# Keep-Passion/ImageStitch

Hardware: AMD Instinct MI355X
Metric: image-pairs/sec (2048x2048 grayscale, SURF+BF) (higher is better)
Workload: dtype f32

## Files before the change

### imagestitch_amd/csrc/api.hip

```cpp
#include "common.h"
#include "canvas_band.h"
#include "ingest_fill.h"
#include "jpeg_huff_core.h"
#include "phase_resolve_math.h"
#include <math.h>
#include <stdarg.h>
#include <stdio.h>
#include <string.h>
#include <algorithm>
#include <map>
#include <tuple>

int fuse_i64_device(vfsms_ctx *ctx, const long long *dA, const long long *dB, int r, int c, int ch, int dx, int dy,
                    uint8_t *d_out, int32_t *info, int method = 0, int levels = 4, int seam_blend = 0, int32_t *d_seam = nullptr);

static thread_local char g_err[512] = "";
void vfsms_set_error(const char *fmt, ...)
{
    va_list ap;
    va_start(ap, fmt);
    vsnprintf(g_err, sizeof(g_err), fmt, ap);
    va_end(ap);
}
extern "C" int vfsms_last_error(char *buf, int buflen)
// ... 747 lines not shown
    if (split > 0) surf_describe_layout(a, &W, cap0);
    if (split < n) surf_describe_layout(a, &W, cap1);
    return a.off;
}
static int surf_run_carve(vfsms_ctx *ctx, SurfRun *run, const SurfSrc *S, int n, const vfsms_surf_params *p, const SurfEnh &enh)
{
    ArenaWalk a = ctx_arena_walk(ctx);
    surf_run_layout(a, run, S, n, p, enh);
    TRY(ctx_arena_commit(ctx, a, "arena exhausted while carving a SURF run"));
    return ctx_copy_small(ctx, run->R.data(), sizeof(RoiDev) * n, run->dR);
}
static int surf_run_prepare(vfsms_ctx *ctx, SurfRun *run, const SurfEnh &enh)
{
    const int n = (int)run->R.size();
    if (enh.mode) {
        TRY(ctx_copy_small(ctx, run->E.data(), sizeof(EnhJob) * n, run->dE));
        TRY(launch_enhance(ctx, run->dE, run->E.data(), n, enh.mode, enh.clip_limit, enh.tile_grid));
    }
    HIP_TRY(hipMemsetAsync(run->cblock, 0, sizeof(int) * 16 * n, ctx->stream));
    return VFSMS_OK;
}
static int surf_run_launch(vfsms_ctx *ctx, const SurfRun &run, int first, int count, bool describe, const vfsms_surf_params *p)
{
    TRY(launch_surf_detect(ctx, run.dR + first, run.R.data() + first, count, p));
    if (describe) TRY(launch_surf_describe(ctx, run.dR + first, run.R.data() + first, count, p));
    return VFSMS_OK;
}
static int surf_run_readback(vfsms_ctx *ctx, SurfRun *run)
{
    run->counters.resize(16 * run->R.size());
    HIP_TRY(hipMemcpyAsync(run->counters.data(), run->cblock, sizeof(int) * run->counters.size(), hipMemcpyDeviceToHost, ctx->stream));
    return VFSMS_OK;
}
static int surf_run_check(const SurfRun &run, const char *who, const char *unit, int index0, int total)
{
    for (size_t i = 0; i < run.R.size(); i++)
        if (run.counters[16 * i + 2] || run.counters[16 * i] > run.R[i].cap) {
            vfsms_set_error("%s: %s %d of %d (%d x %d) exceeded %d keypoint candidates (raise with vfsms_ctx_set_keypoint_capacity)",
                            who, unit, index0 + (int)i, total, run.R[i].h, run.R[i].w, run.R[i].cap);
            return VFSMS_ERR_CAPACITY;
        }
    return VFSMS_OK;
}
static int surf_run_count(const SurfRun &run, int i) { return run.counters[16 * (size_t)i + 1]; }

static int surf_host(vfsms_ctx *ctx, const uint8_t *img, int h, int w, int stride, const vfsms_surf_params *params,
                     float *kps_xy, float *desc, vfsms_keypoint *kps_full, int cap, int *n_out, bool describe)
// ... 2152 lines not shown
```

### imagestitch_amd/csrc/common.h

```cpp
#pragma once
#include <hip/hip_runtime.h>
#include <stdint.h>
#include <condition_variable>
#include <list>
#include <mutex>
#include <string>
#include <unordered_map>
#include <vector>
#include "../../include/vfsms.h"
#include "arena_walk.h"
#include "device_buf.h"

#define VFSMS_MAX_LAYERS 32
#define VFSMS_MAX_WIN 768

#define VFSMS_MAX_OCTAVES 8
#ifdef __HIPCC__
__host__ __device__
#endif
constexpr int vfsms_haar_corner(int size, int k, int c)
{
    constexpr int src[10][4] = { {0, 2, 3, 7}, {3, 2, 6, 7}, {6, 2, 9, 7}, {2, 0, 7, 3}, {2, 3, 7, 6}, {2, 6, 7, 9},
                                 {1, 1, 4, 4}, {5, 1, 8, 4}, {1, 5, 4, 8}, {5, 5, 8, 8} };
    return (2 * size * src[k][c] + 9) / 18;
}
#ifdef __HIPCC__
__host__ __device__
#endif
constexpr int vfsms_haar_src(int k, int c)
{
    constexpr int src[10][4] = { {0, 2, 3, 7}, {3, 2, 6, 7}, {6, 2, 9, 7}, {2, 0, 7, 3}, {2, 3, 7, 6}, {2, 6, 7, 9},
                                 {1, 1, 4, 4}, {5, 1, 8, 4}, {1, 5, 4, 8}, {5, 5, 8, 8} };
    return src[k][c];
// ... 187 lines not shown
void *ctx_arena_alloc(vfsms_ctx *ctx, size_t bytes, size_t align = 256);
ArenaWalk ctx_arena_walk(vfsms_ctx *ctx);
int ctx_arena_commit(vfsms_ctx *ctx, const ArenaWalk &a, const char *what);
int ctx_prepare_surf(vfsms_ctx *ctx, const vfsms_surf_params *p);

struct ShapeRun { int first, count, h, w; };
template <typename Rec>
static std::vector<ShapeRun> shape_runs(const Rec *recs, int n)
{
    std::vector<ShapeRun> runs;
    for (int r = 0; r < n; r++) {
        if (!runs.empty() && runs.back().h == recs[r].h && runs.back().w == recs[r].w) runs.back().count++;
        else runs.push_back(ShapeRun{r, 1, recs[r].h, recs[r].w});
    }
    return runs;
}

void surf_roi_layout(ArenaWalk &a, RoiDev *r, const uint8_t *img, int stride, int h, int w, int cap, const vfsms_surf_params *p);
struct DescWork { int *tickets; DescPlan *plan; DescRec *rec_big, *rec_small; };
void surf_describe_layout(ArenaWalk &a, DescWork *d, size_t capsum);
int launch_integral(vfsms_ctx *ctx, const RoiDev *d_rois, int nrois, int maxh, int maxw);
size_t integral_carry_bytes(int h, int w);
int launch_surf_detect(vfsms_ctx *ctx, const RoiDev *d_rois, const RoiDev *h_rois, int nrois,
                       const vfsms_surf_params *p);
int launch_surf_describe(vfsms_ctx *ctx, const RoiDev *d_rois, const RoiDev *h_rois, int nrois,
                         const vfsms_surf_params *p);
void match_layout(ArenaWalk &a, MatchDev *m, int capq, int dim, int nsplit);
void match_filter_layout(ArenaWalk &a, MatchDev *m, int capq, int capt, int cns);
int launch_max_norm2_d64(vfsms_ctx *ctx, const float *a, int n, unsigned *d_out);
int launch_bf_l2_filtered(vfsms_ctx *ctx, const MatchDev *d_jobs, int njobs, int capq, int capt, int cns);
int launch_bf_l2(vfsms_ctx *ctx, const MatchDev *d_jobs, int njobs, int capq, int nsplit, int dim);
#define BFI_PAD_NORM 0x3fffffff
struct PackJob { const float *src; const int *n_ptr; int8_t *dst; int *nrm; };
int launch_pack_i8_d128(vfsms_ctx *ctx, const PackJob *d_jobs, int njobs, int max_rows);
int launch_bf_i8_d128(vfsms_ctx *ctx, const MatchDev *d_jobs, int njobs, int capq, int nsplit);
int launch_bf_hamming(vfsms_ctx *ctx, const MatchDev *d_jobs, int njobs, int capq, int nsplit, int max_dist);
enum MatchTailKind {
    TAIL_VOTE,
    TAIL_PAIRS,
    TAIL_KNN,
    TAIL_GIVEN_PAIRS
};
struct MatchTail {
    MatchTailKind kind;
    double ratio;
    int max_dist;
    int offset_evaluate;
// ... 196 lines not shown
```

### imagestitch_amd/csrc/surf_kernels.hip

```cpp
#include "common.h"
#include "detmath.h"
#include <math.h>
#include <float.h>
#include <string.h>
#include <stdlib.h>
#include <algorithm>
#include <vector>

#define GAS __attribute__((address_space(1)))
typedef GAS const uint8_t *g_cu8;
typedef GAS const int32_t *g_ci32;
typedef GAS float *g_f32;
typedef GAS const float *g_cf32;
typedef GAS int32_t *g_i32;
__device__ __forceinline__ int cv_round_f(float v) { return (int)rintf(v); }
__device__ __forceinline__ uint8_t round_u8_pos(float v) { return (uint8_t)__float_as_uint(v + 12582912.f); }
__device__ __forceinline__ int cv_round_d(double v) { return (int)rint(v); }
__device__ __forceinline__ int cv_floor_d(double v) { return (int)floor(v); }
__device__ __forceinline__ int cv_ceil_d(double v) { return (int)ceil(v); }

__device__ __forceinline__ int wave_incl_scan(int v)
{
    const int lane = threadIdx.x & 63;
#pragma unroll
    for (int d = 1; d < 64; d <<= 1) {
        int n = __shfl_up(v, d, 64);
        if (lane >= d) v += n;
    }
    return v;
}

#define INT_TH 16
typedef int int4u __attribute__((ext_vector_type(4), aligned(4)));
typedef uint32_t u32u __attribute__((aligned(1)));

__device__ __forceinline__ uint32_t load_px4(g_cu8 row, int x, int w)
{
    const int xa = min(x, w - 4);
    const uint32_t v = *(GAS const u32u *)(row + xa);
    return v >> (8 * (x - xa));
}

__global__ __launch_bounds__(256) void k_integral_bandsum(const RoiDev *rois)
{
    const RoiDev &R = rois[blockIdx.z];
    const int h = R.h, w = R.w, stride = R.stride, ipitch = R.ipitch;
    const int y0 = blockIdx.y * INT_TH;
    const int x = (blockIdx.x * 256 + threadIdx.x) * 4;
    if (y0 >= h || x >= w || w < 4) return;
    const int rows = min(INT_TH, h - y0);
    g_cu8 src = (g_cu8)R.img + (size_t)y0 * stride;
    g_i32 dst = (g_i32)R.icarry + (size_t)blockIdx.y * ipitch + x;
    uint32_t px[INT_TH];
#pragma unroll
    for (int r = 0; r < INT_TH; r++) px[r] = r < rows ? load_px4(src + (size_t)r * stride, x, w) : 0u;
    uint32_t even = 0, odd = 0;
#pragma unroll
    for (int r = 0; r < INT_TH; r++) { even += px[r] & 0x00ff00ffu; odd += (px[r] >> 8) & 0x00ff00ffu; }
    int4u o = {(int)(even & 0xffff), (int)(odd & 0xffff), (int)(even >> 16), (int)(odd >> 16)};
    *(GAS int4u *)dst = o;
}

__global__ __launch_bounds__(256) void k_integral_bandscan(const RoiDev *rois)
{
    const RoiDev &R = rois[blockIdx.y];
    const int ipitch = R.ipitch;
    const int x = blockIdx.x * 256 + threadIdx.x;
    if (x >= ipitch) return;
    const int nb = (R.h + INT_TH - 1) / INT_TH;
    g_i32 c = (g_i32)R.icarry + x;
    int run = 0;
    for (int b0 = 0; b0 < nb; b0 += 16) {
        int v[16];
#pragma unroll
        for (int k = 0; k < 16; k++) v[k] = b0 + k < nb ? c[(size_t)(b0 + k) * ipitch] : 0;
#pragma unroll
        for (int k = 0; k < 16; k++) { if (b0 + k < nb) c[(size_t)(b0 + k) * ipitch] = run; run += v[k]; }
    }
}

__global__ __launch_bounds__(256) void k_integral_final(const RoiDev *rois)
{
    const RoiDev &R = rois[blockIdx.y];
    const int h = R.h, w = R.w, stride = R.stride, ipitch = R.ipitch;
    g_cu8 img = (g_cu8)R.img;
    g_i32 S = (g_i32)R.sum;
    g_ci32 carry = (g_ci32)R.icarry + (size_t)blockIdx.x * ipitch;
    const int y0 = blockIdx.x * INT_TH;
    if (y0 >= h) return;
    const int rows = min(INT_TH, h - y0);
    const int sw = w + 1;
    if (w < 4) {
        if (blockIdx.x == 0 && threadIdx.x == 0) {
            for (int xx = 0; xx < sw; xx++) S[xx] = 0;
            for (int y = 0; y < h; y++) {
                int rs = 0;
                S[(size_t)(y + 1) * sw] = 0;
                for (int xx = 0; xx < w; xx++) { rs += img[(size_t)y * stride + xx]; S[(size_t)(y + 1) * sw + xx + 1] = S[(size_t)y * sw + xx + 1] + rs; }
            }
        }
        return;
    }
    if (blockIdx.x == 0)
        for (int xx = threadIdx.x; xx < sw; xx += 256) S[xx] = 0;
    if (threadIdx.x < rows) S[(size_t)(y0 + 1 + threadIdx.x) * sw] = 0;
    __shared__ int wsum[INT_TH][4];
    const int lane = threadIdx.x & 63, wid = threadIdx.x >> 6;
    g_cu8 src = img + (size_t)y0 * stride;
    int ccarry[INT_TH];
#pragma unroll
    for (int r = 0; r < INT_TH; r++) ccarry[r] = 0;
    for (int c0 = 0; c0 < w; c0 += 1024) {
        const int x = c0 + threadIdx.x * 4;
        const bool in = x < w;
        const int xl = in ? x : 0;
        uint32_t px[INT_TH];
#pragma unroll
        for (int r = 0; r < INT_TH; r++) {
            const uint32_t v = load_px4(src + (size_t)min(r, rows - 1) * stride, xl, w);
            px[r] = (in && r < rows) ? v : 0u;
        }
        int4u C = *(GAS const int4u *)(carry + xl);
        if (!in) { C.x = 0; C.y = 0; C.z = 0; C.w = 0; }
        int tot[INT_TH];
        int run = C.x + C.y + C.z + C.w;
#pragma unroll
        for (int r = 0; r < INT_TH; r++) {
            run += (int)__builtin_amdgcn_sad_u8(px[r], 0u, 0u);
            tot[r] = run;
        }
        int incl[INT_TH];
#pragma unroll
        for (int r = 0; r < INT_TH; r++) incl[r] = tot[r];
#pragma unroll
        for (int d = 1; d < 64; d <<= 1) {
#pragma unroll
            for (int r = 0; r < INT_TH; r++) {
                const int n = __shfl_up(incl[r], d, 64);
                incl[r] += lane >= d ? n : 0;
            }
        }
        if (c0) __syncthreads();
        if (lane == 63) {
// ... 1 lines not shown
            for (int r = 0; r < INT_TH; r++) wsum[r][wid] = incl[r];
        }
        __syncthreads();
        int t0 = C.x, t1 = C.y, t2 = C.z, t3 = C.w;
        g_i32 dst = S + (size_t)(y0 + 1) * sw + 1 + xl;
        const bool whole = x + 3 < w;
#pragma unroll
        for (int r = 0; r < INT_TH; r++) {
            const int4 ws = *reinterpret_cast<const int4 *>(&wsum[r][0]);
            int off = ccarry[r] + incl[r] - tot[r];
            off += wid > 0 ? ws.x : 0; off += wid > 1 ? ws.y : 0; off += wid > 2 ? ws.z : 0;
            ccarry[r] += ws.x + ws.y + ws.z + ws.w;
            t0 += (int)(px[r] & 0xff); t1 += (int)((px[r] >> 8) & 0xff); t2 += (int)((px[r] >> 16) & 0xff); t3 += (int)(px[r] >> 24);
            if (r < rows) {
                int4u o;
                o.x = off + t0; o.y = o.x + t1; o.z = o.y + t2; o.w = o.z + t3;
                if (whole) *(GAS int4u *)(dst + (size_t)r * sw) = o;
                else if (in) { dst[(size_t)r * sw] = o.x; if (x + 1 < w) dst[(size_t)r * sw + 1] = o.y; if (x + 2 < w) dst[(size_t)r * sw + 2] = o.z; }
            }
        }
    }
}

int launch_integral(vfsms_ctx *ctx, const RoiDev *d_rois, int nrois, int maxh, int maxw)
{
    if (nrois <= 0) return VFSMS_OK;
    const int nb = (maxh + INT_TH - 1) / INT_TH;
    hipLaunchKernelGGL(k_integral_bandsum, dim3((maxw + 1023) / 1024, nb, nrois), dim3(256), 0, ctx->stream, d_rois);
    hipLaunchKernelGGL(k_integral_bandscan, dim3((maxw + 3 + 255) / 256, nrois), dim3(256), 0, ctx->stream, d_rois);
    hipLaunchKernelGGL(k_integral_final, dim3(nb, nrois), dim3(256), 0, ctx->stream, d_rois);
    HIP_TRY(hipGetLastError());
    return VFSMS_OK;
}
size_t integral_carry_bytes(int h, int w) { return sizeof(int32_t) * (size_t)((h + INT_TH - 1) / INT_TH) * (size_t)((w + 3) & ~3); }

__device__ __forceinline__ float haar_box(g_ci32 sp, int sw, const LayerPat &P, int k0, int n)
{
    double d = 0;
    for (int k = k0; k < k0 + n; k++) {
        const int dx1 = P.box[k][0], dy1 = P.box[k][1], dx2 = P.box[k][2], dy2 = P.box[k][3];
        int v = sp[dy1 * sw + dx1] + sp[dy2 * sw + dx2] - sp[dy2 * sw + dx1] - sp[dy1 * sw + dx2];
        d += (double)((float)v * P.w[k]);
    }
    return (float)d;
}

__device__ __forceinline__ int cand_class_id(const RoiDev &R, const LayerPat *pats, const Cand &c)
{
    const LayerPat &P = pats[c.layer];
    const int ss = P.step, size = P.size;
    const int sum_i = ss * (c.i - (size / 2) / ss), sum_j = ss * (c.j - (size / 2) / ss);
    g_ci32 sp = (g_ci32)R.sum + (size_t)sum_i * (R.w + 1) + sum_j;
    const float tr = haar_box(sp, R.w + 1, P, 0, 3) + haar_box(sp, R.w + 1, P, 3, 3);
    return (tr > 0) - (tr < 0);
}
// ... 314 lines not shown
        kpt.size = (float)cv_round_f(kpt.size + x2 * ds);
    }
    return ok;
}

__device__ __forceinline__ float nms_max3(float a, float b, float c)
{
    float r;
    asm("v_max3_f32 %0, %1, %2, %3" : "=v"(r) : "v"(a), "v"(b), "v"(c));
    return r;
}
#ifndef NMS_RW
#define NMS_RW 32
#endif
#ifndef NMS_PF
#define NMS_PF 16
#endif
#define NMS_TW 62
#define NMS_TH (4 * NMS_RW)
#define NMS_LOCAL 192
static_assert(NMS_RW % 2 == 0 && NMS_RW <= 256, "k_nms: queue entries keep the row in 8 bits; the queue bound pairs the rows");
static_assert(NMS_TW + 2 == 64, "k_nms: one wave = the evaluated columns + two halo lanes");
struct NmsPlan { int noct; int first[VFSMS_MAX_OCTAVES + 1]; int tiles_x[VFSMS_MAX_OCTAVES]; };

__global__ __launch_bounds__(256) __attribute__((amdgpu_waves_per_eu(8, 8)))
void k_nms(const RoiDev *rois, const LayerPat *pats, int layers_per_octave, int n_middle, NmsPlan plan, float hessianThreshold)
{
    int octave = 0;
    while (octave + 1 < plan.noct && (int)blockIdx.x >= plan.first[octave + 1]) octave++;
    const int tix = (int)blockIdx.x - plan.first[octave];
    const int bx = tix % plan.tiles_x[octave], by = tix / plan.tiles_x[octave];
    const int roi = blockIdx.y / n_middle;
    const int l = 1 + blockIdx.y % n_middle;
    const int li = octave * layers_per_octave + l;
    const RoiDev &R = rois[roi];
    const LayerPat &P = pats[li];
    const int ss = P.step, size = P.size;
    const int lrows = R.h / ss, lcols = R.w / ss;
    const int margin = (pats[li + 1].size / 2) / ss + 1;
    if (pats[li + 1].size > R.h || pats[li + 1].size > R.w) return;
    const int lane = threadIdx.x, wave = __builtin_amdgcn_readfirstlane((int)threadIdx.y), tid = wave * 64 + lane;
    const int j0 = margin - 1 + bx * NMS_TW, i0 = margin + by * NMS_TH;
    if (j0 + 1 >= lcols - margin || i0 >= lrows - margin) return;
    __shared__ unsigned short queue[4][NMS_RW * 16];
    __shared__ int cn, cbase;
    __shared__ Cand local[NMS_LOCAL];
    if (tid == 0) cn = 0;
    __syncthreads();
    g_cf32 d2 = (g_cf32)R.det[li];
    const int st = lcols;
    const int j = j0 + lane;
    const int ia = i0 + wave * NMS_RW;
    int nq = 0;
    if (ia < lrows - margin) {
        const uint32_t joff = (uint32_t)min(j, lcols - 1) * 4u;
        const float thr = (lane >= 1 && lane <= NMS_TW && j < lcols - margin) ? hessianThreshold : __builtin_inff();
// ... 805 lines not shown
                if (p0 + DESC_PASS < cn) __syncthreads();
            }
            DT_MARK(4);
        }
    }
    __syncthreads();
    if (band >= 0) {
        if (threadIdx.x < 21) R.patch[(size_t)k * VFSMS_PATCH_ROW + band * 21 + threadIdx.x] = PATCH[band][threadIdx.x];
    } else {
        for (int o = threadIdx.x; o < 441; o += 256) R.patch[(size_t)k * VFSMS_PATCH_ROW + o] = PATCH[o / 21][o % 21];
    }
    DT_MARK(5);
}

#define DESC_NCLS 4

__device__ __forceinline__ int desc_class(float size)
{
    const float s = size * 1.2f / 9.0f;
    const int win = min((int)((20 + 1) * s), VFSMS_MAX_WIN);
    return win > 256 ? 0 : win > 128 ? 1 : win > 64 ? 2 : 3;
}

__global__ __launch_bounds__(1024) void k_desc_order(const RoiDev *rois)
{
    const RoiDev &R = rois[blockIdx.x];
    const int n = min(R.counters[0], R.cap);
    __shared__ int cnt[DESC_NCLS], base[DESC_NCLS], cur[DESC_NCLS];
    if (threadIdx.x < DESC_NCLS) { cnt[threadIdx.x] = 0; cur[threadIdx.x] = 0; }
    __syncthreads();
    const int lane = threadIdx.x & 63;
    for (int k0 = 0; k0 < n; k0 += 1024) {
        const int k = k0 + threadIdx.x;
        const float size = k < n ? R.kps[k].size : -1.f;
        const int cls = size > 0 ? desc_class(size) : -1;
#pragma unroll
        for (int c = 0; c < DESC_NCLS; c++) {
            const unsigned long long m = __ballot(cls == c);
            if (m && lane == __ffsll((long long)m) - 1) atomicAdd(&cnt[c], __popcll(m));
        }
    }
    __syncthreads();
    if (threadIdx.x == 0) {
        int acc = 0;
        for (int c = 0; c < DESC_NCLS; c++) { base[c] = acc; acc += cnt[c]; R.counters[12 + c] = cnt[c]; }
    }
    __syncthreads();
    for (int k0 = 0; k0 < n; k0 += 1024) {
        const int k = k0 + threadIdx.x;
        const float size = k < n ? R.kps[k].size : -1.f;
        const int cls = size > 0 ? desc_class(size) : -1;
#pragma unroll
        for (int c = 0; c < DESC_NCLS; c++) {
            const unsigned long long m = __ballot(cls == c);
            if (!m) continue;
            const int leader = __ffsll((long long)m) - 1;
            int start = 0;
            if (lane == leader) start = atomicAdd(&cur[c], __popcll(m));
            start = __shfl(start, leader, 64);
            if (cls == c) R.order[base[c] + start + __popcll(m & ((1ull << lane) - 1))] = k;
        }
    }
}

#define DESC_HEADS DESC_PLAN_HEADS
#define DESC_HEAD_STRIDE 64

__global__ __launch_bounds__(256) void k_desc_plan(const RoiDev *rois, int nrois, DescPlan *plan, int big_grid)
{
    __shared__ int c[VFSMS_MAX_ROIS][4];
    for (int e = threadIdx.x; e < nrois * 4; e += 256) c[e >> 2][e & 3] = rois[e >> 2].counters[12 + (e & 3)];
    __syncthreads();
    if (threadIdx.x == 0) {
        int acc = 0, total = 0;
        for (int q = 0; q < DESC_HEADS; q++) {
            plan->big_start[q] = acc;
            for (int r = q; r < nrois; r += DESC_HEADS) { plan->seg_base[r][0] = acc; acc += c[r][0]; }
            plan->big_n0[q] = acc - plan->big_start[q];
            for (int r = q; r < nrois; r += DESC_HEADS) {
                plan->seg_base[r][1] = acc; acc += c[r][1];
                plan->seg_base[r][2] = acc; acc += c[r][2];
            }
            plan->big_tickets[q] = acc - plan->big_start[q];
        }
        total = acc;
        const int split = total < big_grid * 48 ? 21 : 1;
        plan->split = split;
        for (int q = 0; q < DESC_HEADS; q++) plan->big_tickets[q] += (split - 1) * plan->big_n0[q];
        acc = 0;
        for (int q = 0; q < DESC_HEADS; q++) {
            plan->small_start[q] = acc;
            for (int r = q; r < nrois; r += DESC_HEADS) { plan->seg_base[r][3] = acc; acc += c[r][3]; }
            plan->small_tickets[q] = acc - plan->small_start[q];
        }
    }
}
// ... 122 lines not shown
__global__ __launch_bounds__(256, DESC_SMALL_WGS) void k_describe_small(const RoiDev *rois, const DescPlan *plan, const DescRec *recs, int *counter,
                                                                 const AreaRec *area_tab, int upright)
{
    __shared__ SmallLds L[4];
    if (threadIdx.x < 4) L[threadIdx.x].rec_win = -1;
    __syncthreads();
    const int lane = threadIdx.x & 63, wave = __builtin_amdgcn_readfirstlane((int)(threadIdx.x >> 6));
    int head = 0;
    for (;;) {
        int slot = -1;
        if (lane == 0)
            while (head < DESC_HEADS) {
                const int q = (blockIdx.x + head) & (DESC_HEADS - 1);
                const int n = plan->small_tickets[q];
                const int t = n > 0 ? atomicAdd(counter + q * DESC_HEAD_STRIDE, 1) : 0;
                if (t < n) { slot = plan->small_start[q] + t; break; }
                head++;
            }
        slot = __builtin_amdgcn_readfirstlane(slot);
        head = __builtin_amdgcn_readfirstlane(head);
        if (slot < 0) break;
        const DescRec rec = load_rec_uniform(recs + slot);
        describe_small(rois[rec.roi], area_tab, rec, upright, L[wave]);
    }
}

__global__ __launch_bounds__(256) void k_pair_rows(const RoiDev *rois)
{
    const RoiDev &R = rois[blockIdx.z];
    const int y = blockIdx.y, x = (blockIdx.x * 256 + threadIdx.x) * 4;
    if (y >= R.h || x >= R.w) return;
    g_cu8 r0 = (g_cu8)R.img + (size_t)y * R.stride + x, r1 = (g_cu8)R.img + (size_t)min(y + 1, R.h - 1) * R.stride + x;
    GAS uint16_t *dst = (GAS uint16_t *)R.pair + (size_t)y * R.w + x;
    if (x + 4 <= R.w) {
        const uint32_t a = *(GAS const u32u *)r0, b = *(GAS const u32u *)r1;
#pragma unroll
        for (int k = 0; k < 4; k++) dst[k] = (uint16_t)(((a >> (8 * k)) & 0xff) | (((b >> (8 * k)) & 0xff) << 8));
    } else {
        for (int k = 0; x + k < R.w; k++) dst[k] = (uint16_t)(r0[k] | (r1[k] << 8));
    }
}

#ifndef DESC_WGS
#define DESC_WGS 6
#endif
__global__ __launch_bounds__(256, DESC_WGS) void k_describe(const RoiDev *rois, const DescPlan *plan, const DescRec *recs, int *counter, const SurfTables *T,
                                                  const AreaRec *area_tab, int extended, int upright)
{
    __shared__ int s_slot, s_band;
    int head = 0;
#ifdef VFSMS_DESC_TIMING
    unsigned long long tq = clock64();
#endif
    for (;;) {
        __syncthreads();
        if (threadIdx.x == 0) {
            int slot = -1, band = -1;
            const int split = plan->split;
            while (head < DESC_HEADS) {
                const int q = (blockIdx.x + head) & (DESC_HEADS - 1);
                const int n = plan->big_tickets[q];
                const int t = n > 0 ? atomicAdd(counter + q * DESC_HEAD_STRIDE, 1) : 0;
// ... 1 lines not shown
                    const int n0 = plan->big_n0[q];
                    if (t < n0 * split) { slot = plan->big_start[q] + t / split; band = split > 1 ? t % split : -1; }
                    else slot = plan->big_start[q] + n0 + (t - n0 * split);
                    break;
                }
                head++;
            }
            s_slot = slot; s_band = band;
        }
        __syncthreads();
        const int slot = __builtin_amdgcn_readfirstlane(s_slot), band = __builtin_amdgcn_readfirstlane(s_band);
        if (slot < 0) break;
#ifdef VFSMS_DESC_TIMING
        if (threadIdx.x == 0) atomicAdd(&g_desc_cycles[6], clock64() - tq);
#endif
        const DescRec rec = load_rec_uniform(recs + slot);
        describe_one(rois[rec.roi], T, area_tab, rec, extended, upright, band);
#ifdef VFSMS_DESC_TIMING
        tq = clock64();
#endif
    }
}

__global__ __launch_bounds__(1024) void k_keep_scan(const RoiDev *rois)
{
    const RoiDev &R = rois[blockIdx.x];
    const int n = min(R.counters[0], R.cap);
    __shared__ int wsum[16];
    __shared__ int carry;
    if (threadIdx.x == 0) carry = 0;
    __syncthreads();
    const int lane = threadIdx.x & 63, wid = threadIdx.x >> 6;
    for (int base = 0; base < n; base += 1024) {
        int idx = base + threadIdx.x;
        int keep = (idx < n) ? (R.kps[idx].size > 0 ? 1 : 0) : 0;
        int incl = wave_incl_scan(keep);
        if (lane == 63) wsum[wid] = incl;
        __syncthreads();
        int off = carry;
        for (int k = 0; k < wid; k++) off += wsum[k];
        if (idx < n) R.keep_pos[idx] = keep ? (off + incl - 1) : -1;
        __syncthreads();
        if (threadIdx.x == 1023) carry = off + incl;
        __syncthreads();
    }
    if (threadIdx.x == 0) R.counters[1] = carry;
}


__global__ __launch_bounds__(256) void k_desc_tail(const RoiDev *rois, const SurfTables *T, int extended)
{
    const RoiDev &R = rois[blockIdx.y];
    const int n = min(R.counters[0], R.cap);
    const int k0 = blockIdx.x * 16;
    if (k0 >= n) return;
    const int dsize = extended ? 128 : 64;
    __shared__ uint32_t P32[16][VFSMS_PATCH_ROW / 4];
    __shared__ float vec[16][128];
    __shared__ float scl[16];
    __shared__ float DWs[400];
    for (int i = threadIdx.x; i < 400; i += 256) DWs[i] = T->DW[i];
    {
        const uint32_t __attribute__((address_space(1))) *src =
            (const uint32_t __attribute__((address_space(1))) *)(R.patch + (size_t)k0 * VFSMS_PATCH_ROW);
        const int rows = min(16, n - k0);
        for (int i = threadIdx.x; i < rows * (VFSMS_PATCH_ROW / 4); i += 256) (&P32[0][0])[i] = src[i];
    }
    __syncthreads();
    const int kk = threadIdx.x >> 4, c = threadIdx.x & 15, k = k0 + kk;
    const int pos = k < n ? R.keep_pos[k] : -1;
    if (pos >= 0) {
        const uint8_t *P = (const uint8_t *)&P32[kk][0];
// ... 55 lines not shown
    for (int o = 0; o < p->n_octaves; o++) {
        const size_t n = (size_t)(h / step) * (w / step);
        for (int l = 0; l < lpo; l++) r->det[o * lpo + l] = a.take<float>(n);
        step *= 2;
    }
    r->cand = a.take<Cand>(cap);
    r->kps = a.take<vfsms_keypoint>(cap);
    r->patch = a.take<uint8_t>((size_t)cap * VFSMS_PATCH_ROW);
    r->keep_pos = a.take<int>(cap);
    r->order = a.take<int>(cap);
    r->kps_xy = a.take<float>(2 * (size_t)cap);
    r->desc = a.take<float>((size_t)cap * (p->extended ? 128 : 64));
    r->kps_out = a.take<vfsms_keypoint>(cap);
}

void surf_describe_layout(ArenaWalk &a, DescWork *d, size_t capsum)
{
    d->tickets = a.take<int>(2 * DESC_HEADS * DESC_HEAD_STRIDE);
    d->plan = a.take<DescPlan>(1);
    d->rec_big = a.take<DescRec>(capsum);
    d->rec_small = a.take<DescRec>(capsum);
}

int launch_surf_detect(vfsms_ctx *ctx, const RoiDev *d_rois, const RoiDev *h_rois, int nrois,
                       const vfsms_surf_params *p)
{
    if (nrois <= 0) return VFSMS_OK;
    const int lpo = p->n_octave_layers + 2;
    int maxcap = 0;
    for (int r = 0; r < nrois; r++) maxcap = h_rois[r].cap > maxcap ? h_rois[r].cap : maxcap;
    const std::vector<ShapeRun> runs = shape_runs(h_rois, nrois);
    {
        ProfScope ps(ctx, "integral");
        for (const ShapeRun &q : runs) TRY(launch_integral(ctx, d_rois + q.first, q.count, q.h, q.w));
    }
    {
        ProfScope ps(ctx, "hessian");
        static const bool generic = getenv("VFSMS_HESSIAN_GENERIC") && atoi(getenv("VFSMS_HESSIAN_GENERIC")) != 0;
        for (const ShapeRun &q : runs) {
            const RoiDev *dq = d_rois + q.first;
            int step = 1, o = 0;
            if (lpo == 5) {
                for (; o < p->n_octaves && o < 2; o++) {
                    const int lrows = q.h / step, lcols = q.w / step;
                    if (lrows > 0 && lcols > 0) {
                        if (o == 0)
                            hipLaunchKernelGGL((k_hessian_lds<1, 64, 4>), dim3((lcols + 63) / 64, (lrows + 15) / 16, q.count), dim3(64, 4), 0, ctx->stream, dq, ctx->d_layers.as<LayerPat>(), lpo, o);
                        else
                            hipLaunchKernelGGL((k_hessian_lds<2, 32, HESS_O1_WAVES>), dim3((lcols + 31) / 32, (lrows + 15) / 16, q.count), dim3(64, HESS_O1_WAVES), 0, ctx->stream, dq, ctx->d_layers.as<LayerPat>(), lpo, o);
                    }
                    step *= 2;
                }
            }
            static const bool rows2 = !(getenv("VFSMS_HESSIAN_ROWS2") && atoi(getenv("VFSMS_HESSIAN_ROWS2")) == 0);
            if (lpo == 5 && o == 2 && o < p->n_octaves && rows2 && !generic) {
                const int s0 = 36;
                if (q.h >= s0 && q.w >= s0) {
// ... 2 lines not shown
                                       tiles_i, tiles_j, q.count);
                }
                o++; step *= 2;
            }
            HessPlan plan; plan.o0 = o; plan.noct = 0; plan.first[0] = 0;
            for (; o < p->n_octaves && plan.noct < VFSMS_MAX_OCTAVES; o++) {
                const int lrows = q.h / step, lcols = q.w / step;
                const int tx = (lcols + 63) / 64, ty = (lrows + 3) / 4;
                plan.tiles_x[plan.noct] = tx > 0 ? tx : 1;
                plan.first[plan.noct + 1] = plan.first[plan.noct] + tx * ty;
                plan.noct++;
                step *= 2;
            }
            if (plan.noct > 0 && plan.first[plan.noct] > 0) {
                if (lpo == 5 && plan.o0 >= 2 && plan.o0 + plan.noct <= 4 && !generic)
                    hipLaunchKernelGGL(k_hessian_coarse, dim3((unsigned)plan.first[plan.noct] * lpo * q.count), dim3(64, 4), 0, ctx->stream, dq, ctx->d_layers.as<LayerPat>(), lpo, plan, q.count);
                else
                    hipLaunchKernelGGL(k_hessian, dim3((unsigned)plan.first[plan.noct] * lpo * q.count), dim3(64, 4), 0, ctx->stream, dq, ctx->d_layers.as<LayerPat>(), lpo, plan, q.count);
            }
        }
    }
    {
        ProfScope ps(ctx, "nms");
        for (const ShapeRun &q : runs) {
            NmsPlan plan; plan.noct = 0; plan.first[0] = 0;
            int step = 1;
            for (int o = 0; o < p->n_octaves && o < VFSMS_MAX_OCTAVES; o++) {
                const int lrows = q.h / step, lcols = q.w / step;
                const int tx = (lcols + NMS_TW - 1) / NMS_TW, ty = (lrows + NMS_TH - 1) / NMS_TH;
                plan.tiles_x[o] = tx > 0 ? tx : 1;
                plan.first[o + 1] = plan.first[o] + tx * ty;
                plan.noct = o + 1;
                step *= 2;
            }
            if (plan.noct > 0 && plan.first[plan.noct] > 0)
                hipLaunchKernelGGL(k_nms, dim3(plan.first[plan.noct], q.count * p->n_octave_layers), dim3(64, 4), 0, ctx->stream, d_rois + q.first,
                                   ctx->d_layers.as<LayerPat>(), lpo, p->n_octave_layers, plan, p->hessian_threshold);
        }
    }
    {
        ProfScope ps(ctx, "sort");
        static const bool n2sort = getenv("VFSMS_SORT_N2") && atoi(getenv("VFSMS_SORT_N2")) != 0;
        int mincap = maxcap;
        for (int r = 0; r < nrois; r++) mincap = h_rois[r].cap < mincap ? h_rois[r].cap : mincap;
        if (n2sort || mincap < SORT_BUCKETS) hipLaunchKernelGGL(k_rank_sort, dim3((maxcap + 63) / 64, nrois), dim3(256), 0, ctx->stream, d_rois, ctx->d_layers.as<LayerPat>());
        else {
            hipLaunchKernelGGL(k_bucket_sort, dim3(nrois), dim3(1024), 0, ctx->stream, d_rois);
            hipLaunchKernelGGL(k_bucket_rank, dim3((maxcap + 255) / 256, nrois), dim3(256), 0, ctx->stream, d_rois, ctx->d_layers.as<LayerPat>());
        }
    }
    HIP_TRY(hipGetLastError());
    return VFSMS_OK;
}


int ctx_prepare_area_tab(vfsms_ctx *ctx)
{
    if (ctx->d_area_tab) return VFSMS_OK;
    std::vector<AreaRec> tab((size_t)(VFSMS_MAX_WIN + 1) * AREA_RECS);
    memset(tab.data(), 0, sizeof(AreaRec) * tab.size());
// ... 30 lines not shown
        }
        if (nmax > 40) { vfsms_set_error("internal: INTER_AREA run of window %d", win); return VFSMS_ERR_UNSUPPORTED; }
        rec[21].j0 = nmin; rec[21].n = nmax; rec[21].a0 = fast ? 1.f / (iscale * iscale) : 1.f;
        rec[21].mode = !fast ? 0 : iscale == 2 ? 2 : 1;
    }
    for (int win = 0; win < dsz; win++) memcpy(tab.data() + (size_t)win * AREA_RECS, tab.data() + (size_t)dsz * AREA_RECS, sizeof(AreaRec) * AREA_RECS);
    TRY(ctx->d_area_tab.reserve(sizeof(AreaRec) * tab.size(), ctx->stream));
    HIP_TRY(hipMemcpy(ctx->d_area_tab.as<void>(), tab.data(), sizeof(AreaRec) * tab.size(), hipMemcpyHostToDevice));
    return VFSMS_OK;
}

int launch_surf_describe(vfsms_ctx *ctx, const RoiDev *d_rois, const RoiDev *h_rois, int nrois,
                         const vfsms_surf_params *p)
{
    if (nrois <= 0) return VFSMS_OK;
    if (nrois > VFSMS_MAX_ROIS) { vfsms_set_error("more than %d ROIs in one batch", VFSMS_MAX_ROIS); return VFSMS_ERR_CAPACITY; }
    TRY(ctx_prepare_area_tab(ctx));
    int maxcap = 0;
    for (int r = 0; r < nrois; r++) maxcap = h_rois[r].cap > maxcap ? h_rois[r].cap : maxcap;
    {
        ProfScope ps(ctx, "orientation");
        hipLaunchKernelGGL(k_orientation, dim3((maxcap + ORI_KP - 1) / ORI_KP, nrois), dim3(ORI_KP * 128), 0, ctx->stream, d_rois, ctx->d_tables.as<SurfTables>(), p->upright);
    }
    {
        ProfScope ps(ctx, "compact");
        hipLaunchKernelGGL(k_keep_scan, dim3(nrois), dim3(1024), 0, ctx->stream, d_rois);
    }
    {
        ProfScope ps(ctx, "describe");
        size_t capsum = 0;
        for (int r = 0; r < nrois; r++) capsum += (size_t)h_rois[r].cap;
        ArenaWalk a = ctx_arena_walk(ctx); DescWork W;
        surf_describe_layout(a, &W, capsum);
        TRY(ctx_arena_commit(ctx, a, "arena exhausted (descriptor work list)"));
        HIP_TRY(hipMemsetAsync(W.tickets, 0, sizeof(int) * 2 * DESC_HEADS * DESC_HEAD_STRIDE, ctx->stream));
        for (const ShapeRun &q : shape_runs(h_rois, nrois))
            hipLaunchKernelGGL(k_pair_rows, dim3((q.w + 1023) / 1024, q.h, q.count), dim3(256), 0, ctx->stream, d_rois + q.first);
        hipLaunchKernelGGL(k_desc_order, dim3(nrois), dim3(1024), 0, ctx->stream, d_rois);
        hipLaunchKernelGGL(k_desc_plan, dim3(1), dim3(256), 0, ctx->stream, d_rois, nrois, W.plan, 256 * DESC_WGS);
        hipLaunchKernelGGL(k_desc_recs, dim3((maxcap + 255) / 256, nrois), dim3(256), 0, ctx->stream, d_rois, W.plan, W.rec_big, W.rec_small, p->upright);
        hipLaunchKernelGGL(k_describe, dim3(256 * DESC_WGS), dim3(256), 0, ctx->stream, d_rois, W.plan, W.rec_big, W.tickets,
                           ctx->d_tables.as<SurfTables>(), ctx->d_area_tab.as<AreaRec>(), p->extended, p->upright);
        hipLaunchKernelGGL(k_describe_small, dim3(256 * DESC_SMALL_WGS), dim3(256), 0, ctx->stream, d_rois, W.plan, W.rec_small,
                           W.tickets + DESC_HEADS * DESC_HEAD_STRIDE, ctx->d_area_tab.as<AreaRec>(), p->upright);
        hipLaunchKernelGGL(k_desc_tail, dim3((maxcap + 15) / 16, nrois), dim3(256), 0, ctx->stream, d_rois, ctx->d_tables.as<SurfTables>(), p->extended);
    }
    HIP_TRY(hipGetLastError());
    return VFSMS_OK;
}
```

Before: 2471.

## Merge shape runs into single launches and fuse pair-rows and descriptor prep kernels

Adds a ShapeTiles mapping so the integral and NMS kernels cover up to four ROI shape runs with one flat 1-D grid each, instead of one launch per shape. The paired-row image (pair) is now written inside the final integral pass when description follows, which removes the separate k_pair_rows kernel and its extra read of the image. The keep-scan, descriptor ordering, plan and ticket memset are folded into one k_desc_prepare kernel, using a last-block-done atomic counter. This cuts launch count and memory traffic, at the cost of extra index arithmetic per block and a global atomic handoff that depends on counters[3] starting at zero.

After: 2512 (median of 3 runs). +1.6%, better.

```diff
diff --git a/imagestitch_amd/csrc/api.hip b/imagestitch_amd/csrc/api.hip
--- a/imagestitch_amd/csrc/api.hip
+++ b/imagestitch_amd/csrc/api.hip
@@ -793,7 +793,7 @@
 }
 static int surf_run_launch(vfsms_ctx *ctx, const SurfRun &run, int first, int count, bool describe, const vfsms_surf_params *p)
 {
-    TRY(launch_surf_detect(ctx, run.dR + first, run.R.data() + first, count, p));
+    TRY(launch_surf_detect(ctx, run.dR + first, run.R.data() + first, count, p, describe));
     if (describe) TRY(launch_surf_describe(ctx, run.dR + first, run.R.data() + first, count, p));
     return VFSMS_OK;
 }
diff --git a/imagestitch_amd/csrc/common.h b/imagestitch_amd/csrc/common.h
--- a/imagestitch_amd/csrc/common.h
+++ b/imagestitch_amd/csrc/common.h
@@ -9,6 +9,7 @@
 #include <vector>
 #include "../../include/vfsms.h"
 #include "arena_walk.h"
+#include "shape_tiles.h"
 #include "device_buf.h"
 
 #define VFSMS_MAX_LAYERS 32
@@ -242,7 +243,7 @@
 int launch_integral(vfsms_ctx *ctx, const RoiDev *d_rois, int nrois, int maxh, int maxw);
 size_t integral_carry_bytes(int h, int w);
 int launch_surf_detect(vfsms_ctx *ctx, const RoiDev *d_rois, const RoiDev *h_rois, int nrois,
-                       const vfsms_surf_params *p);
+                       const vfsms_surf_params *p, bool write_pair);
 int launch_surf_describe(vfsms_ctx *ctx, const RoiDev *d_rois, const RoiDev *h_rois, int nrois,
                          const vfsms_surf_params *p);
 void match_layout(ArenaWalk &a, MatchDev *m, int capq, int dim, int nsplit);
diff --git a/imagestitch_amd/csrc/shape_tiles.h b/imagestitch_amd/csrc/shape_tiles.h
--- /dev/null
+++ b/imagestitch_amd/csrc/shape_tiles.h
@@ -0,0 +1,40 @@
+#pragma once
+#ifndef SHAPE_TILES_HD
+#ifdef __HIPCC__
+#define SHAPE_TILES_HD __host__ __device__ __forceinline__
+#else
+#define SHAPE_TILES_HD inline
+#endif
+#endif
+
+#define SHAPE_TILES_MAX 4
+struct ShapeTiles {
+    int nruns;
+    int first[SHAPE_TILES_MAX], count[SHAPE_TILES_MAX], h[SHAPE_TILES_MAX], w[SHAPE_TILES_MAX];
+    unsigned per_roi[SHAPE_TILES_MAX], block0[SHAPE_TILES_MAX + 1];
+};
+struct ShapeTilePos { int run, roi; unsigned inner; int h, w; };
+
+template <typename Run, typename Blocks>
+inline bool shape_tiles_build(ShapeTiles &T, const Run *runs, int nruns, Blocks blocks)
+{
+    if (nruns > SHAPE_TILES_MAX) return false;
+    T = ShapeTiles{};
+    T.nruns = nruns;
+    for (int r = 0; r < nruns; r++) {
+        T.first[r] = runs[r].first; T.count[r] = runs[r].count; T.h[r] = runs[r].h; T.w[r] = runs[r].w;
+        T.per_roi[r] = (unsigned)blocks(runs[r].h, runs[r].w);
+        T.block0[r + 1] = T.block0[r] + T.per_roi[r] * (unsigned)runs[r].count;
+    }
+    return true;
+}
+
+SHAPE_TILES_HD ShapeTilePos shape_tiles_locate(const ShapeTiles &T, unsigned L)
+{
+    int run = 0;
+#pragma unroll
+    for (int r = 1; r < SHAPE_TILES_MAX; r++)
+        if (r < T.nruns && L >= T.block0[r]) run = r;
+    const unsigned local = L - T.block0[run], per = T.per_roi[run];
+    return ShapeTilePos{run, T.first[run] + (int)(local / per), local % per, T.h[run], T.w[run]};
+}
diff --git a/imagestitch_amd/csrc/surf_kernels.hip b/imagestitch_amd/csrc/surf_kernels.hip
--- a/imagestitch_amd/csrc/surf_kernels.hip
+++ b/imagestitch_amd/csrc/surf_kernels.hip
@@ -41,16 +41,19 @@
     return v >> (8 * (x - xa));
 }
 
-__global__ __launch_bounds__(256) void k_integral_bandsum(const RoiDev *rois)
-{
-    const RoiDev &R = rois[blockIdx.z];
+__global__ __launch_bounds__(256) void k_integral_bandsum(const RoiDev *rois, ShapeTiles T)
+{
+    const ShapeTilePos q = shape_tiles_locate(T, blockIdx.x);
+    const RoiDev &R = rois[q.roi];
     const int h = R.h, w = R.w, stride = R.stride, ipitch = R.ipitch;
-    const int y0 = blockIdx.y * INT_TH;
-    const int x = (blockIdx.x * 256 + threadIdx.x) * 4;
+    const unsigned gx = (unsigned)(q.w + 1023) / 1024u;
+    const int band = (int)(q.inner / gx);
+    const int y0 = band * INT_TH;
+    const int x = ((int)(q.inner % gx) * 256 + threadIdx.x) * 4;
     if (y0 >= h || x >= w || w < 4) return;
     const int rows = min(INT_TH, h - y0);
     g_cu8 src = (g_cu8)R.img + (size_t)y0 * stride;
-    g_i32 dst = (g_i32)R.icarry + (size_t)blockIdx.y * ipitch + x;
+    g_i32 dst = (g_i32)R.icarry + (size_t)band * ipitch + x;
     uint32_t px[INT_TH];
 #pragma unroll
     for (int r = 0; r < INT_TH; r++) px[r] = r < rows ? load_px4(src + (size_t)r * stride, x, w) : 0u;
@@ -61,11 +64,12 @@
     *(GAS int4u *)dst = o;
 }
 
-__global__ __launch_bounds__(256) void k_integral_bandscan(const RoiDev *rois)
-{
-    const RoiDev &R = rois[blockIdx.y];
+__global__ __launch_bounds__(256) void k_integral_bandscan(const RoiDev *rois, ShapeTiles T)
+{
+    const ShapeTilePos q = shape_tiles_locate(T, blockIdx.x);
+    const RoiDev &R = rois[q.roi];
     const int ipitch = R.ipitch;
-    const int x = blockIdx.x * 256 + threadIdx.x;
+    const int x = (int)q.inner * 256 + threadIdx.x;
     if (x >= ipitch) return;
     const int nb = (R.h + INT_TH - 1) / INT_TH;
     g_i32 c = (g_i32)R.icarry + x;
@@ -79,19 +83,33 @@
     }
 }
 
-__global__ __launch_bounds__(256) void k_integral_final(const RoiDev *rois)
-{
-    const RoiDev &R = rois[blockIdx.y];
+typedef uint32_t pair4u __attribute__((ext_vector_type(2), aligned(2)));
+__device__ __forceinline__ pair4u pair_px4(uint32_t a, uint32_t b)
+{
+    pair4u v = {(a & 0xffu) | ((b & 0xffu) << 8) | ((a & 0xff00u) << 8) | ((b & 0xff00u) << 16),
+                ((a >> 16) & 0xffu) | ((b >> 8) & 0xff00u) | ((a >> 8) & 0xff0000u) | (b & 0xff000000u)};
+    return v;
+}
+template <bool PAIR>
+__global__ __launch_bounds__(256) void k_integral_final(const RoiDev *rois, ShapeTiles T)
+{
+    const ShapeTilePos q = shape_tiles_locate(T, blockIdx.x);
+    const RoiDev &R = rois[q.roi];
+    const int band = (int)q.inner;
     const int h = R.h, w = R.w, stride = R.stride, ipitch = R.ipitch;
     g_cu8 img = (g_cu8)R.img;
     g_i32 S = (g_i32)R.sum;
-    g_ci32 carry = (g_ci32)R.icarry + (size_t)blockIdx.x * ipitch;
-    const int y0 = blockIdx.x * INT_TH;
+    GAS uint16_t *pair = (GAS uint16_t *)R.pair;
+    g_ci32 carry = (g_ci32)R.icarry + (size_t)band * ipitch;
+    const int y0 = band * INT_TH;
     if (y0 >= h) return;
     const int rows = min(INT_TH, h - y0);
     const int sw = w + 1;
     if (w < 4) {
-        if (blockIdx.x == 0 && threadIdx.x == 0) {
+        if (band == 0 && threadIdx.x == 0) {
+            if (PAIR)
+                for (int y = 0; y < h; y++)
+                    for (int xx = 0; xx < w; xx++) pair[(size_t)y * w + xx] = (uint16_t)(img[(size_t)y * stride + xx] | (img[(size_t)min(y + 1, h - 1) * stride + xx] << 8));
             for (int xx = 0; xx < sw; xx++) S[xx] = 0;
             for (int y = 0; y < h; y++) {
                 int rs = 0;
@@ -101,7 +119,7 @@
         }
         return;
     }
-    if (blockIdx.x == 0)
+    if (band == 0)
         for (int xx = threadIdx.x; xx < sw; xx += 256) S[xx] = 0;
     if (threadIdx.x < rows) S[(size_t)(y0 + 1 + threadIdx.x) * sw] = 0;
     __shared__ int wsum[INT_TH][4];
@@ -119,6 +137,24 @@
         for (int r = 0; r < INT_TH; r++) {
             const uint32_t v = load_px4(src + (size_t)min(r, rows - 1) * stride, xl, w);
             px[r] = (in && r < rows) ? v : 0u;
+        }
+        if (PAIR && in) {
+            const uint32_t below = load_px4(img + (size_t)min(y0 + rows, h - 1) * stride, xl, w);
+            GAS uint16_t *pd = pair + (size_t)y0 * w + x;
+            const bool whole4 = x + 3 < w;
+#pragma unroll
+            for (int r = 0; r < INT_TH; r++) {
+                if (r < rows) {
+                    const uint32_t b = r + 1 < INT_TH ? (r + 1 < rows ? px[r + 1 < INT_TH ? r + 1 : r] : below) : below;
+                    const pair4u v = pair_px4(px[r], b);
+                    if (whole4) *(GAS pair4u *)(pd + (size_t)r * w) = v;
+                    else {
+                        pd[(size_t)r * w] = (uint16_t)v.x;
+                        if (x + 1 < w) pd[(size_t)r * w + 1] = (uint16_t)(v.x >> 16);
+                        if (x + 2 < w) pd[(size_t)r * w + 2] = (uint16_t)v.y;
+                    }
+                }
+            }
         }
         int4u C = *(GAS const int4u *)(carry + xl);
         if (!in) { C.x = 0; C.y = 0; C.z = 0; C.w = 0; }
@@ -166,15 +202,30 @@
     }
 }
 
-int launch_integral(vfsms_ctx *ctx, const RoiDev *d_rois, int nrois, int maxh, int maxw)
-{
-    if (nrois <= 0) return VFSMS_OK;
-    const int nb = (maxh + INT_TH - 1) / INT_TH;
-    hipLaunchKernelGGL(k_integral_bandsum, dim3((maxw + 1023) / 1024, nb, nrois), dim3(256), 0, ctx->stream, d_rois);
-    hipLaunchKernelGGL(k_integral_bandscan, dim3((maxw + 3 + 255) / 256, nrois), dim3(256), 0, ctx->stream, d_rois);
-    hipLaunchKernelGGL(k_integral_final, dim3(nb, nrois), dim3(256), 0, ctx->stream, d_rois);
+template <typename Blocks, typename Launch>
+static void shape_tiles_launch(const ShapeRun *runs, int nruns, Blocks blocks, Launch launch)
+{
+    ShapeTiles T;
+    if (shape_tiles_build(T, runs, nruns, blocks) && T.block0[T.nruns] > 0) launch(T);
+}
+static int launch_integral_runs(vfsms_ctx *ctx, const RoiDev *d_rois, const ShapeRun *runs, int nruns, bool pair)
+{
+    auto bands = [](int h) { return (h + INT_TH - 1) / INT_TH; };
+    shape_tiles_launch(runs, nruns, [&](int h, int w) { return ((w + 1023) / 1024) * bands(h); }, [&](const ShapeTiles &T) {
+        hipLaunchKernelGGL(k_integral_bandsum, dim3(T.block0[T.nruns]), dim3(256), 0, ctx->stream, d_rois, T); });
+    shape_tiles_launch(runs, nruns, [&](int h, int w) { return (w + 3 + 255) / 256; }, [&](const ShapeTiles &T) {
+        hipLaunchKernelGGL(k_integral_bandscan, dim3(T.block0[T.nruns]), dim3(256), 0, ctx->stream, d_rois, T); });
+    shape_tiles_launch(runs, nruns, [&](int h, int w) { return bands(h); }, [&](const ShapeTiles &T) {
+        if (pair) hipLaunchKernelGGL(k_integral_final<true>, dim3(T.block0[T.nruns]), dim3(256), 0, ctx->stream, d_rois, T);
+        else hipLaunchKernelGGL(k_integral_final<false>, dim3(T.block0[T.nruns]), dim3(256), 0, ctx->stream, d_rois, T); });
     HIP_TRY(hipGetLastError());
     return VFSMS_OK;
+}
+int launch_integral(vfsms_ctx *ctx, const RoiDev *d_rois, int nrois, int maxh, int maxw)
+{
+    if (nrois <= 0) return VFSMS_OK;
+    const ShapeRun one{0, nrois, maxh, maxw};
+    return launch_integral_runs(ctx, d_rois, &one, 1, false);
 }
 size_t integral_carry_bytes(int h, int w) { return sizeof(int32_t) * (size_t)((h + INT_TH - 1) / INT_TH) * (size_t)((w + 3) & ~3); }
 
@@ -535,16 +586,21 @@
 static_assert(NMS_RW % 2 == 0 && NMS_RW <= 256, "k_nms: queue entries keep the row in 8 bits; the queue bound pairs the rows");
 static_assert(NMS_TW + 2 == 64, "k_nms: one wave = the evaluated columns + two halo lanes");
 struct NmsPlan { int noct; int first[VFSMS_MAX_OCTAVES + 1]; int tiles_x[VFSMS_MAX_OCTAVES]; };
+struct NmsPlans { NmsPlan p[SHAPE_TILES_MAX]; };
 
 __global__ __launch_bounds__(256) __attribute__((amdgpu_waves_per_eu(8, 8)))
-void k_nms(const RoiDev *rois, const LayerPat *pats, int layers_per_octave, int n_middle, NmsPlan plan, float hessianThreshold)
-{
+void k_nms(const RoiDev *rois, const LayerPat *pats, int layers_per_octave, int n_middle, NmsPlans plans, ShapeTiles T, float hessianThreshold)
+{
+    const ShapeTilePos pos = shape_tiles_locate(T, blockIdx.x);
+    const NmsPlan &plan = plans.p[pos.run];
+    const int ntiles = plan.first[plan.noct];
+    const int tile = (int)(pos.inner % (unsigned)ntiles);
     int octave = 0;
-    while (octave + 1 < plan.noct && (int)blockIdx.x >= plan.first[octave + 1]) octave++;
-    const int tix = (int)blockIdx.x - plan.first[octave];
+    while (octave + 1 < plan.noct && tile >= plan.first[octave + 1]) octave++;
+    const int tix = tile - plan.first[octave];
     const int bx = tix % plan.tiles_x[octave], by = tix / plan.tiles_x[octave];
-    const int roi = blockIdx.y / n_middle;
-    const int l = 1 + blockIdx.y % n_middle;
+    const int roi = pos.roi;
+    const int l = 1 + (int)(pos.inner / (unsigned)ntiles);
     const int li = octave * layers_per_octave + l;
     const RoiDev &R = rois[roi];
     const LayerPat &P = pats[li];
@@ -1396,26 +1452,42 @@
     return win > 256 ? 0 : win > 128 ? 1 : win > 64 ? 2 : 3;
 }
 
-__global__ __launch_bounds__(1024) void k_desc_order(const RoiDev *rois)
+#define DESC_HEADS DESC_PLAN_HEADS
+#define DESC_HEAD_STRIDE 64
+
+__global__ __launch_bounds__(1024) void k_desc_prepare(const RoiDev *rois, int nrois, DescPlan *plan, int *tickets, int nticket_ints, int big_grid)
 {
     const RoiDev &R = rois[blockIdx.x];
     const int n = min(R.counters[0], R.cap);
+    __shared__ int wsum[16];
+    __shared__ int carry, last;
     __shared__ int cnt[DESC_NCLS], base[DESC_NCLS], cur[DESC_NCLS];
+    if (threadIdx.x == 0) carry = 0;
     if (threadIdx.x < DESC_NCLS) { cnt[threadIdx.x] = 0; cur[threadIdx.x] = 0; }
     __syncthreads();
-    const int lane = threadIdx.x & 63;
+    const int lane = threadIdx.x & 63, wid = threadIdx.x >> 6;
     for (int k0 = 0; k0 < n; k0 += 1024) {
-        const int k = k0 + threadIdx.x;
-        const float size = k < n ? R.kps[k].size : -1.f;
+        const int idx = k0 + threadIdx.x;
+        const float size = idx < n ? R.kps[idx].size : -1.f;
+        const int keep = size > 0 ? 1 : 0;
         const int cls = size > 0 ? desc_class(size) : -1;
 #pragma unroll
         for (int c = 0; c < DESC_NCLS; c++) {
             const unsigned long long m = __ballot(cls == c);
             if (m && lane == __ffsll((long long)m) - 1) atomicAdd(&cnt[c], __popcll(m));
         }
-    }
-    __syncthreads();
+        const int incl = wave_incl_scan(keep);
+        if (lane == 63) wsum[wid] = incl;
+        __syncthreads();
+        int off = carry;
+        for (int k = 0; k < wid; k++) off += wsum[k];
+        if (idx < n) R.keep_pos[idx] = keep ? (off + incl - 1) : -1;
+        __syncthreads();
+        if (threadIdx.x == 1023) carry = off + incl;
+        __syncthreads();
+    }
     if (threadIdx.x == 0) {
+        R.counters[1] = carry;
         int acc = 0;
         for (int c = 0; c < DESC_NCLS; c++) { base[c] = acc; acc += cnt[c]; R.counters[12 + c] = cnt[c]; }
     }
@@ -1435,17 +1507,20 @@
             if (cls == c) R.order[base[c] + start + __popcll(m & ((1ull << lane) - 1))] = k;
         }
     }
-}
-
-#define DESC_HEADS DESC_PLAN_HEADS
-#define DESC_HEAD_STRIDE 64
-
-__global__ __launch_bounds__(256) void k_desc_plan(const RoiDev *rois, int nrois, DescPlan *plan, int big_grid)
-{
+    int *done = rois[0].counters + 3;
+    if (threadIdx.x == 0) {
+        __threadfence();
+        last = atomicAdd(done, 1) == nrois - 1;
+        __threadfence();
+    }
+    __syncthreads();
+    if (!last) return;
     __shared__ int c[VFSMS_MAX_ROIS][4];
-    for (int e = threadIdx.x; e < nrois * 4; e += 256) c[e >> 2][e & 3] = rois[e >> 2].counters[12 + (e & 3)];
+    for (int e = threadIdx.x; e < nrois * 4; e += 1024) c[e >> 2][e & 3] = __hip_atomic_load(rois[e >> 2].counters + 12 + (e & 3), __ATOMIC_RELAXED, __HIP_MEMORY_SCOPE_AGENT);
+    for (int e = threadIdx.x; e < nticket_ints; e += 1024) tickets[e] = 0;
     __syncthreads();
     if (threadIdx.x == 0) {
+        *done = 0;
         int acc = 0, total = 0;
         for (int q = 0; q < DESC_HEADS; q++) {
             plan->big_start[q] = acc;
@@ -1614,22 +1689,6 @@
         if (slot < 0) break;
         const DescRec rec = load_rec_uniform(recs + slot);
         describe_small(rois[rec.roi], area_tab, rec, upright, L[wave]);
-    }
-}
-
-__global__ __launch_bounds__(256) void k_pair_rows(const RoiDev *rois)
-{
-    const RoiDev &R = rois[blockIdx.z];
-    const int y = blockIdx.y, x = (blockIdx.x * 256 + threadIdx.x) * 4;
-    if (y >= R.h || x >= R.w) return;
-    g_cu8 r0 = (g_cu8)R.img + (size_t)y * R.stride + x, r1 = (g_cu8)R.img + (size_t)min(y + 1, R.h - 1) * R.stride + x;
-    GAS uint16_t *dst = (GAS uint16_t *)R.pair + (size_t)y * R.w + x;
-    if (x + 4 <= R.w) {
-        const uint32_t a = *(GAS const u32u *)r0, b = *(GAS const u32u *)r1;
-#pragma unroll
-        for (int k = 0; k < 4; k++) dst[k] = (uint16_t)(((a >> (8 * k)) & 0xff) | (((b >> (8 * k)) & 0xff) << 8));
-    } else {
-        for (int k = 0; x + k < R.w; k++) dst[k] = (uint16_t)(r0[k] | (r1[k] << 8));
     }
 }
 
@@ -1677,32 +1736,6 @@
     }
 }
 
-__global__ __launch_bounds__(1024) void k_keep_scan(const RoiDev *rois)
-{
-    const RoiDev &R = rois[blockIdx.x];
-    const int n = min(R.counters[0], R.cap);
-    __shared__ int wsum[16];
-    __shared__ int carry;
-    if (threadIdx.x == 0) carry = 0;
-    __syncthreads();
-    const int lane = threadIdx.x & 63, wid = threadIdx.x >> 6;
-    for (int base = 0; base < n; base += 1024) {
-        int idx = base + threadIdx.x;
-        int keep = (idx < n) ? (R.kps[idx].size > 0 ? 1 : 0) : 0;
-        int incl = wave_incl_scan(keep);
-        if (lane == 63) wsum[wid] = incl;
-        __syncthreads();
-        int off = carry;
-        for (int k = 0; k < wid; k++) off += wsum[k];
-        if (idx < n) R.keep_pos[idx] = keep ? (off + incl - 1) : -1;
-        __syncthreads();
-        if (threadIdx.x == 1023) carry = off + incl;
-        __syncthreads();
-    }
-    if (threadIdx.x == 0) R.counters[1] = carry;
-}
-
-
 __global__ __launch_bounds__(256) void k_desc_tail(const RoiDev *rois, const SurfTables *T, int extended)
 {
     const RoiDev &R = rois[blockIdx.y];
@@ -1804,17 +1837,26 @@
     d->rec_small = a.take<DescRec>(capsum);
 }
 
+static bool shape_merge_enabled()
+{
+    static const bool on = !(getenv("VFSMS_SHAPE_MERGE") && atoi(getenv("VFSMS_SHAPE_MERGE")) == 0);
+    return on;
+}
+
 int launch_surf_detect(vfsms_ctx *ctx, const RoiDev *d_rois, const RoiDev *h_rois, int nrois,
-                       const vfsms_surf_params *p)
+                       const vfsms_surf_params *p, bool write_pair)
 {
     if (nrois <= 0) return VFSMS_OK;
     const int lpo = p->n_octave_layers + 2;
     int maxcap = 0;
     for (int r = 0; r < nrois; r++) maxcap = h_rois[r].cap > maxcap ? h_rois[r].cap : maxcap;
     const std::vector<ShapeRun> runs = shape_runs(h_rois, nrois);
+    const int per = shape_merge_enabled() && (int)runs.size() <= SHAPE_TILES_MAX ? (int)runs.size() : 1;
+    const LayerPat *pats = ctx->d_layers.as<LayerPat>();
+    hipStream_t st = ctx->stream;
     {
         ProfScope ps(ctx, "integral");
-        for (const ShapeRun &q : runs) TRY(launch_integral(ctx, d_rois + q.first, q.count, q.h, q.w));
+        for (size_t g = 0; g < runs.size(); g += per) TRY(launch_integral_runs(ctx, d_rois, runs.data() + g, per, write_pair));
     }
     {
         ProfScope ps(ctx, "hessian");
@@ -1863,20 +1905,24 @@
     }
     {
         ProfScope ps(ctx, "nms");
-        for (const ShapeRun &q : runs) {
-            NmsPlan plan; plan.noct = 0; plan.first[0] = 0;
-            int step = 1;
-            for (int o = 0; o < p->n_octaves && o < VFSMS_MAX_OCTAVES; o++) {
-                const int lrows = q.h / step, lcols = q.w / step;
-                const int tx = (lcols + NMS_TW - 1) / NMS_TW, ty = (lrows + NMS_TH - 1) / NMS_TH;
-                plan.tiles_x[o] = tx > 0 ? tx : 1;
-                plan.first[o + 1] = plan.first[o] + tx * ty;
-                plan.noct = o + 1;
-                step *= 2;
-            }
-            if (plan.noct > 0 && plan.first[plan.noct] > 0)
-                hipLaunchKernelGGL(k_nms, dim3(plan.first[plan.noct], q.count * p->n_octave_layers), dim3(64, 4), 0, ctx->stream, d_rois + q.first,
-                                   ctx->d_layers.as<LayerPat>(), lpo, p->n_octave_layers, plan, p->hessian_threshold);
+        for (size_t g = 0; g < runs.size(); g += per) {
+            const ShapeRun *rg = runs.data() + g;
+            NmsPlans plans; memset(&plans, 0, sizeof(plans));
+            for (int r = 0; r < per; r++) {
+                NmsPlan &plan = plans.p[r];
+                int step = 1;
+                for (int o = 0; o < p->n_octaves && o < VFSMS_MAX_OCTAVES; o++) {
+                    const int lrows = rg[r].h / step, lcols = rg[r].w / step;
+                    const int tx = (lcols + NMS_TW - 1) / NMS_TW, ty = (lrows + NMS_TH - 1) / NMS_TH;
+                    plan.tiles_x[o] = tx > 0 ? tx : 1;
+                    plan.first[o + 1] = plan.first[o] + tx * ty;
+                    plan.noct = o + 1;
+                    step *= 2;
+                }
+            }
+            int r = 0;
+            shape_tiles_launch(rg, per, [&](int, int) { const NmsPlan &q = plans.p[r++]; return q.noct > 0 ? q.first[q.noct] * p->n_octave_layers : 0; }, [&](const ShapeTiles &T) {
+                hipLaunchKernelGGL(k_nms, dim3(T.block0[T.nruns]), dim3(64, 4), 0, st, d_rois, pats, lpo, p->n_octave_layers, plans, T, p->hessian_threshold); });
         }
     }
     {
@@ -1953,22 +1999,17 @@
         ProfScope ps(ctx, "orientation");
         hipLaunchKernelGGL(k_orientation, dim3((maxcap + ORI_KP - 1) / ORI_KP, nrois), dim3(ORI_KP * 128), 0, ctx->stream, d_rois, ctx->d_tables.as<SurfTables>(), p->upright);
     }
+    size_t capsum = 0;
+    for (int r = 0; r < nrois; r++) capsum += (size_t)h_rois[r].cap;
+    ArenaWalk a = ctx_arena_walk(ctx); DescWork W;
+    surf_describe_layout(a, &W, capsum);
+    TRY(ctx_arena_commit(ctx, a, "arena exhausted (descriptor work list)"));
     {
         ProfScope ps(ctx, "compact");
-        hipLaunchKernelGGL(k_keep_scan, dim3(nrois), dim3(1024), 0, ctx->stream, d_rois);
+        hipLaunchKernelGGL(k_desc_prepare, dim3(nrois), dim3(1024), 0, ctx->stream, d_rois, nrois, W.plan, W.tickets, 2 * DESC_HEADS * DESC_HEAD_STRIDE, 256 * DESC_WGS);
     }
     {
         ProfScope ps(ctx, "describe");
-        size_t capsum = 0;
-        for (int r = 0; r < nrois; r++) capsum += (size_t)h_rois[r].cap;
-        ArenaWalk a = ctx_arena_walk(ctx); DescWork W;
-        surf_describe_layout(a, &W, capsum);
-        TRY(ctx_arena_commit(ctx, a, "arena exhausted (descriptor work list)"));
-        HIP_TRY(hipMemsetAsync(W.tickets, 0, sizeof(int) * 2 * DESC_HEADS * DESC_HEAD_STRIDE, ctx->stream));
-        for (const ShapeRun &q : shape_runs(h_rois, nrois))
-            hipLaunchKernelGGL(k_pair_rows, dim3((q.w + 1023) / 1024, q.h, q.count), dim3(256), 0, ctx->stream, d_rois + q.first);
-        hipLaunchKernelGGL(k_desc_order, dim3(nrois), dim3(1024), 0, ctx->stream, d_rois);
-        hipLaunchKernelGGL(k_desc_plan, dim3(1), dim3(256), 0, ctx->stream, d_rois, nrois, W.plan, 256 * DESC_WGS);
         hipLaunchKernelGGL(k_desc_recs, dim3((maxcap + 255) / 256, nrois), dim3(256), 0, ctx->stream, d_rois, W.plan, W.rec_big, W.rec_small, p->upright);
         hipLaunchKernelGGL(k_describe, dim3(256 * DESC_WGS), dim3(256), 0, ctx->stream, d_rois, W.plan, W.rec_big, W.tickets,
                            ctx->d_tables.as<SurfTables>(), ctx->d_area_tab.as<AreaRec>(), p->extended, p->upright);
```
